# AechPro/Prism

Hardware: NVIDIA B200
Metric: PER sampled transitions/s (4 new steps ingested -> sample -> 3-step gather -> DQN update -> priority write-back, per learner iteration) (higher is better)
Workload: dtype f32

## Files before the change

### include/prism_b200.h

```cpp
#ifndef PRISM_B200_H
#define PRISM_B200_H

#include <stdint.h>

#ifdef __cplusplus
extern "C" {
#endif

#define PB_ABI_VERSION 2

enum {
    PB_OK = 0,
    PB_E_ARG = -1,
    PB_E_CAPACITY = -2,
    PB_E_UNSUPPORTED = -3,
    PB_E_POOL = -4
};

enum {
    PB_ST_EMPTY = 1,
    PB_ST_PSUM_NONPOS = 2,
    PB_ST_PMIN_NONPOS = 4
};

// ... 157 lines not shown
int pb_ens_q_loss_total(int B, int A, int K, const float *q_cur, const float *q_next_online, const float *q_next_target,
                        const long long *action, const float *ret, const float *gdn, const uint8_t *nonterminal,
                        float loss_weight, const float *row_weight, float grad_scale, float *loss_out, float *grad_q_cur,
                        const float *dist, float q_scale, const float *q_offset, float *total_out, float *td_out,
                        unsigned int *ticket, void *stream);

int pb_ids_select(int N, int A, int K, int Nq, const float *q, const float *z, float lambda,
                  float eps, float rho_lower_bound, long long *action_out, float *scores_out,
                  void *stream);

int pb_greedy_select(int N, int A, int K, const float *q, long long *action_out, void *stream);

#define PB_ADAM_MAX_PARTIALS 4096
int pb_pack_grads_parity(int n_tensors, const long long *table, float scale, float *flat,
                         const unsigned long long *epoch, long long stride, float *partial_scratch,
                         long long *step_count, int *n_partials_out_h, void *stream);
int pb_pack_grads(int n_tensors, const long long *table, float scale, float *flat,
                  float *partial_scratch, long long *step_count, int *n_partials_out_h,
                  void *stream);
int pb_grad_sumsq(long long n, const float *grad, float *partial_scratch, long long *step_count,
                  int *n_partials_out_h, void *stream);
int pb_adam_clip_apply(long long n, float *param, const float *grad, float *exp_avg,
                       float *exp_avg_sq, const long long *step_count, float lr, float beta1,
                       float beta2, float adam_eps, float max_grad_norm,
                       const float *partial_scratch, int n_partials, float *norm_out,
                       void *stream);
long long pb_adam_fused_max_n(void);
int pb_adam_fused_step(int n_tensors, const long long *table, float scale, long long n, float *param, float *grad,
                       float *exp_avg, float *exp_avg_sq, long long *step_count, float lr, float beta1, float beta2,
                       float adam_eps, float max_grad_norm, float *partial_scratch, float *norm_out, void *stream);
int pb_adam_clip_step(long long n, float *param, const float *grad, float *exp_avg, float *exp_avg_sq,
                      long long *step_count, float lr, float beta1, float beta2, float adam_eps,
                      float max_grad_norm, float *norm_out, float *partial_scratch, void *stream);

#define PB_OPT_ADAM 0
#define PB_OPT_RMSPROP 1
#define PB_OPT_RMSPROP_CENTERED 2
#define PB_OPT_SGD 3
long long pb_opt_fused_max_n(int rule);
int pb_opt_fused_step(int rule, int n_tensors, const long long *table, float scale, long long n, float *param, float *grad,
                      float *m, float *v, long long *step_count, float lr, float h1, float h2, float eps,
                      float max_grad_norm, float *partial_scratch, float *norm_out, void *stream);
int pb_opt_clip_apply(int rule, long long n, float *param, const float *grad, float *m, float *v,
                      const long long *step_count, float lr, float h1, float h2, float eps, float max_grad_norm,
                      const float *partial_scratch, int n_partials, float *norm_out, void *stream);

int pb_conv3x3_relu_supported(int H, int W, int C, int OC);
int pb_conv3x3_relu_fwd(int B, int H, int W, int C, int OC, const float *x, const float *w,
                        const float *bias, float *out, void *stream);
int pb_conv3x3_relu_bwd_groups(int B);
int pb_conv3x3_relu_bwd(int B, int H, int W, int C, int OC, const float *x, const float *out,
                        const float *dout, float *partial_scratch, float *dw, float *db,
                        void *stream);

int pb_linear_fwd(int K, int M, int N, int J, const float *X, long long x_head_stride, const float *W,
                  const float *b, int act, float *Y, void *stream);
int pb_linear_bwd_input(int K, int M, int N, int J, const float *dY, const float *Ymask, const float *W,
                        int sum_heads, float *dX, void *stream);
int pb_linear_bwd_weight(int K, int M, int N, int J, const float *dY, const float *Ymask, const float *X,
                         long long x_head_stride, float *dW, float *db, void *stream);
int pb_gemm_trace(int enable, unsigned long long *out, int n_out);

int pb_tc_gemm_supported(int M, int N, int K, long long lda, long long ldb, long long ldc);
int pb_tc_gemm(int batch, int kbatches, int M, int N, int K,
               const float *A, int a_major, long long lda, long long a_bs,
               const float *B, int b_major, long long ldb, long long b_bs,
               const float *bias, long long bias_bs, int act,
               const float *mul, int mul_rows, long long ld_mul,
               float *C, long long ldc, long long c_bs,
               float *workspace, long long workspace_floats, int split_mode, void *stream);
int pb_linear_fwd_tc_supported(int M, int N, int J);
int pb_linear_fwd_tc(int K, int M, int N, int J, const float *X, long long x_head_stride, const float *W,
                     const float *b, int act, float *Y, void *stream);

int pb_iqn_phi_bwd(int n, int B, int F, const float *dh, const float *phi, const float *x, float *dpre, float *dx,
                   float *dbias_partial, void *stream);

#define PB_PEER_MAX 8
typedef struct pb_peer_group {
    int world, rank;
    float *grad[PB_PEER_MAX];
    float *reduced[PB_PEER_MAX];
    unsigned long long *flags[PB_PEER_MAX];
    double *norm_parts[PB_PEER_MAX];
    unsigned char *state[PB_PEER_MAX];
    unsigned long long *epoch;
    unsigned int *status;
    unsigned long long timeout_ns;
    long long grad_stride;
} pb_peer_group;
int pb_peer_alloc(long long bytes, void **ptr);
int pb_peer_free(void *ptr);
int pb_optimizer_preload(void);
int pb_peer_preload(void);
int pb_peer_export(const void *ptr, void *handle64);
int pb_peer_open(const void *handle64, void **ptr);
int pb_peer_close(void *ptr);
int pb_peer_barrier(const pb_peer_group *g, void *stream);
int pb_peer_state_allgather(const pb_peer_group *g, const void *state64, void *all_state_out, void *stream);
long long pb_peer_slice(long long n, int world);
int pb_peer_reduce_scatter(const pb_peer_group *g, long long n, float *partial_scratch, long long *step_count, void *stream);
int pb_peer_pull_sum(const pb_peer_group *g, long long n, float *partial_scratch, long long *step_count,
                     int *n_partials_out_h, void *stream);
int pb_peer_adam(const pb_peer_group *g, long long n, float *param, float *exp_avg, float *exp_avg_sq,
                 const long long *step_count, float lr, float beta1, float beta2, float adam_eps, float max_grad_norm,
                 float *norm_out, float *grad_out, void *stream);
// ... 78 lines not shown
```

### prism_b200/_lib.py

```python
import ctypes as C
import os

from . import build as _build

_LIB = None


class PbError(RuntimeError):
    pass


class pb_per_state(C.Structure):
    _fields_ = [
        ("len", C.c_longlong), ("seq", C.c_longlong), ("max_priority", C.c_float), ("p_sum", C.c_float),
        ("p_min", C.c_float), ("status", C.c_int), ("batch_max", C.c_float), ("owned_lo", C.c_int),
        ("owned_n", C.c_int), ("pad", C.c_int * 5),
    ]


class pb_tree(C.Structure):
    _fields_ = [
        ("sum", C.c_void_p), ("min", C.c_void_p), ("owner", C.c_void_p), ("counters", C.c_void_p),
        ("state", C.c_void_p),
        ("capacity", C.c_longlong), ("size", C.c_longlong), ("alpha", C.c_float), ("eps_f32", C.c_float),
# ... 41 lines not shown
    "pb_error_string": [_I],
    "pb_launch_count": [],
    "pb_event_create": [C.POINTER(C.c_void_p)],
    "pb_event_destroy": [_P],
    "pb_event_record": [_P, _P],
    "pb_event_synchronize": [_P],
    "pb_stream_wait_event": [_P, _P],
    "pb_copy_h2d_async": [_P, _P, _LL, _P],
    "pb_staged_copy_submit": [_P, _P, _P, _P, _LL, _P, _P],
    "pb_copy_d2h_async": [_P, _P, _LL, _P],
    "pb_copy_d2d_async": [_P, _P, _LL, _P],
    "pb_tree_layout": [_LL, C.POINTER(C.c_longlong), C.POINTER(C.c_longlong), C.POINTER(C.c_longlong),
                       C.POINTER(C.c_longlong), C.POINTER(C.c_int)],
    "pb_tree_init": [_TREE, _P],
    "pb_tree_export": [_TREE, _P, _P, _P],
    "pb_tree_trace": [_I, _P, _I],
    "pb_gemm_trace": [_I, _P, _I],
    "pb_tree_sample_batches": [_TREE, _LL, _LL, _P, _I, _F, _P, _P, _P, _P],
    "pb_tree_build": [_TREE, _P, _LL, _P],
    "pb_tree_stats": [_TREE, _P],
    "pb_tree_set_leaves": [_TREE, _LL, _P, _P, _I, _P],
    "pb_tree_update_priority": [_TREE, _LL, _P, _P, _I, _P],
    "pb_tree_extend": [_TREE, _LL, _P, _P],
    "pb_tree_scan": [_TREE, _LL, _P, _P, _P],
    "pb_tree_sample": [_TREE, _LL, _P, _I, _F, _P, _P, _P, _P],
    "pb_tree_sample_global": [_TREE, _I, _I, _P, _LL, _P, _F, _P, _P, _P, _P],
    "pb_store_extend_plan": [_LL, _LL, _I, _LL, _LL, _P, _P, _P, _P, _P, _P],
    "pb_store_scatter": [_STORE, _LL, _P, _P, _P, _P],
    "pb_select_copy_f64": [_P, _P, _P, _P, _LL, _LL, _P],
    "pb_store_scatter_dbuf": [_STORE, _LL, _P, _P, _P, _P, _P, _P, _P, _P],
    "pb_store_gather": [_STORE, _LL, _P, _P, _P, _P, _P, _P, _P, _P],
    "pb_store_nstep": [_STORE, _LL, _P, _P, _P, _P, _P, _P, _P],
    "pb_iqn_cos_basis": [_LL, _I, _P, _P, _P],
    "pb_iqn_qh_loss": [_I, _I, _I, _I, _P, _P, _P, _P, _P, _P, _P, _P, _F, _F, _P, _F, _P, _P, _P],
    "pb_ens_q_loss": [_I, _I, _I, _P, _P, _P, _P, _P, _P, _P, _F, _P, _F, _P, _P, _P],
    "pb_ens_q_loss_total": [_I, _I, _I, _P, _P, _P, _P, _P, _P, _P, _F, _P, _F, _P, _P, _P, _F, _P, _P, _P, _P, _P],
    "pb_ids_select": [_I, _I, _I, _I, _P, _P, _F, _F, _F, _P, _P, _P],
    "pb_greedy_select": [_I, _I, _I, _P, _P, _P],
    "pb_adam_clip_step": [_LL, _P, _P, _P, _P, _P, _F, _F, _F, _F, _F, _P, _P, _P],
    "pb_adam_fused_max_n": [],
    "pb_adam_fused_step": [_I, _P, _F, _LL, _P, _P, _P, _P, _P, _F, _F, _F, _F, _F, _P, _P, _P],
    "pb_pack_grads": [_I, _P, _F, _P, _P, _P, _P, _P],
    "pb_pack_grads_parity": [_I, _P, _F, _P, _P, _LL, _P, _P, _P, _P],
    "pb_grad_sumsq": [_LL, _P, _P, _P, _P, _P],
    "pb_adam_clip_apply": [_LL, _P, _P, _P, _P, _P, _F, _F, _F, _F, _F, _P, _I, _P, _P],
    "pb_opt_fused_max_n": [_I],
    "pb_opt_fused_step": [_I, _I, _P, _F, _LL, _P, _P, _P, _P, _P, _F, _F, _F, _F, _F, _P, _P, _P],
    "pb_opt_clip_apply": [_I, _LL, _P, _P, _P, _P, _P, _F, _F, _F, _F, _F, _P, _I, _P, _P],
    "pb_loss_combine": [_I, _P, _P, _P, _F, _P, _P, _P, _P],
    "pb_conv3x3_relu_supported": [_I, _I, _I, _I],
    "pb_conv3x3_relu_fwd": [_I, _I, _I, _I, _I, _P, _P, _P, _P, _P],
    "pb_conv3x3_relu_bwd_groups": [_I],
    "pb_conv3x3_relu_bwd": [_I, _I, _I, _I, _I, _P, _P, _P, _P, _P, _P, _P],
    "pb_linear_fwd": [_I, _I, _I, _I, _P, _LL, _P, _P, _I, _P, _P],
    "pb_peer_alloc": [_LL, C.POINTER(C.c_void_p)],
    "pb_peer_free": [_P],
    "pb_peer_preload": [],
    "pb_optimizer_preload": [],
    "pb_peer_export": [_P, _P],
    "pb_peer_open": [_P, C.POINTER(C.c_void_p)],
    "pb_peer_close": [_P],
    "pb_peer_barrier": [_PEER, _P],
    "pb_peer_state_allgather": [_PEER, _P, _P, _P],
    "pb_peer_slice": [_LL, _I],
    "pb_peer_reduce_scatter": [_PEER, _LL, _P, _P, _P],
    "pb_peer_pull_sum": [_PEER, _LL, _P, _P, C.POINTER(C.c_int), _P],
    "pb_peer_adam": [_PEER, _LL, _P, _P, _P, _P, _F, _F, _F, _F, _F, _P, _P, _P],
    "pb_peer_allreduce_adam_max_n": [],
    "pb_peer_allreduce_adam": [_PEER, _LL, _P, _P, _P, _P, _F, _F, _F, _F, _F, _P, _P, _P],
    "pb_peer_allreduce_opt_max_n": [_I],
    "pb_peer_allreduce_opt": [_I, _PEER, _LL, _P, _P, _P, _P, _F, _F, _F, _F, _F, _P, _P, _P],
    "pb_peer_opt": [_I, _PEER, _LL, _P, _P, _P, _P, _F, _F, _F, _F, _F, _P, _P, _P],
    "pb_peer_state_put": [_PEER, _P, _P],
    "pb_peer_trace": [_I, _P, _I],
    "pb_tree_sample_global_peer": [_TREE, _PEER, _LL, _P, _F, _P, _P, _P, _P],
    "pb_uniform_init": [_P, _LL, _LL, _I, _P],
    "pb_uniform_extend": [_P, _LL, _LL, _P],
    "pb_uniform_sample": [_P, _LL, _P, _I, _P, _P, _P],
    "pb_uniform_sample_global": [_P, _I, _I, _P, _LL, _P, _P, _P, _P, _P],
    "pb_uniform_sample_global_peer": [_P, _PEER, _LL, _P, _P, _P, _P, _P],
    "pb_layer_norm_supported": [_LL, _I],
    "pb_layer_norm_bwd_blocks": [_LL, _I],
    "pb_layer_norm_fwd": [_LL, _I, _F, _P, _P, _P, _P, _P, _P, _P],
    "pb_layer_norm_bwd": [_LL, _I, _P, _P, _P, _P, _P, _P, _P, _P, _P, _P],
    "pb_layer_norm_grouped_fwd": [_I, _LL, _LL, _I, _F, _P, _P, _P, _P, _P, _P, _P],
    "pb_layer_norm_grouped_bwd_blocks": [_I, _LL, _I],
    "pb_layer_norm_grouped_bwd": [_I, _LL, _LL, _I, _P, _P, _P, _P, _P, _P, _P, _P, _P, _P],
    "pb_narrow_linear_supported": [_LL, _I, _I],
    "pb_narrow_linear_bwd_blocks": [_LL],
    "pb_narrow_linear_fwd": [_I, _LL, _I, _I, _P, _LL, _P, _P, _P, _P],
    "pb_narrow_linear_bwd": [_I, _LL, _I, _I, _P, _LL, _P, _P, _P, _P, _P, _P, _P],
    "pb_narrow_linear_bwd_reduce": [_I, _LL, _I, _I, _P, _P, _P, _P],
    "pb_sum_heads": [_I, _LL, _P, _P, _P],
    "pb_iqn_draw_cos_basis": [_LL, _I, _P, _P, _P, _P],
    "pb_relu_bwd_bias_strips": [_LL],
    "pb_relu_bwd_bias": [_I, _LL, _I, _P, _P, _P, _P, _P, _P],
    "pb_theil_chunks": [_LL],
    "pb_theil_fwd": [_I, _I, _I, _P, _P, _P, _P, _P],
    "pb_theil_bwd": [_I, _I, _I, _P, _P, _P, _P, _P],
    "pb_iqn_phi_bwd": [_I, _I, _I, _P, _P, _P, _P, _P, _P, _P],
    "pb_tc_gemm_supported": [_I, _I, _I, _LL, _LL, _LL],
    "pb_tc_gemm": [_I, _I, _I, _I, _I, _P, _I, _LL, _LL, _P, _I, _LL, _LL, _P, _LL, _I, _P, _I, _LL, _P, _LL, _LL, _P, _LL, _I, _P],
    "pb_linear_fwd_tc_supported": [_I, _I, _I],
    "pb_linear_fwd_tc": [_I, _I, _I, _I, _P, _LL, _P, _P, _I, _P, _P],
    "pb_linear_bwd_input": [_I, _I, _I, _I, _P, _P, _P, _I, _P, _P],
    "pb_linear_bwd_weight": [_I, _I, _I, _I, _P, _P, _P, _LL, _P, _P, _P],
# ... 62 lines not shown
```

### prism_b200/agents/ops.py

```python
import collections

import torch

from .. import _lib

ROUTES = collections.Counter()


def route_counts(reset=False):
    out = dict(ROUTES)
    if reset:
        ROUTES.clear()
    return out


def fallthrough_count():
    return sum(v for k, v in ROUTES.items() if k.startswith("fallthrough"))


def _c(t, dtype=torch.float32):
    if t.dtype != dtype:
        t = t.to(dtype)
    return t if t.is_contiguous() else t.contiguous()

# ... 639 lines not shown
        _lib.require_cuda(ref, "tables")
        lib, stream, dev = _lib.load(), _stream(ref), ref.device
        B = action.numel()
        action_c, ret_c, gamma_c = _c(action, torch.int64).view(-1), _c(ret).view(-1), _c(gamma).view(-1)
        nt = None if nonterm is None else nonterm.contiguous().view(-1).view(torch.uint8)
        w_c = None if w is None else _c(w).view(-1)
        dist = mse = gz = gq = None
        if z_cur is not None:
            zc = _c(z_cur)
            dist = torch.empty(B, dtype=torch.float32, device=dev)
            gz = torch.empty_like(zc)
            _lib.check(lib.pb_iqn_qh_loss(B, T, Tp, zc.shape[-1], zc.data_ptr(), _c(tau).view(-1).data_ptr(),
                                          _c(z_on).data_ptr(), _c(z_tg).data_ptr(), action_c.data_ptr(),
                                          ret_c.data_ptr(), gamma_c.data_ptr(), _lib.ptr(nt), float(kappa),
                                          float(dist_weight), _lib.ptr(w_c), 1.0 / B, dist.data_ptr(), gz.data_ptr(),
                                          stream), "pb_iqn_qh_loss")
        total = torch.empty((), dtype=torch.float32, device=dev)
        td = torch.empty(B, dtype=torch.float32, device=dev)
        if q_cur is not None:
            qc = _c(q_cur)
            K, _, A = qc.shape
            mse = torch.empty(B, dtype=torch.float32, device=dev)
            gq = torch.empty_like(qc)
            _lib.check(lib.pb_ens_q_loss_total(B, A, K, qc.data_ptr(), _c(q_on).data_ptr(), _c(q_tg).data_ptr(),
                                               action_c.data_ptr(), ret_c.data_ptr(), gamma_c.data_ptr(), _lib.ptr(nt), 1.0,
                                               _lib.ptr(w_c), float(q_weight) / B, mse.data_ptr(), gq.data_ptr(),
                                               _lib.ptr(dist), float(q_weight), _lib.ptr(q_offset), total.data_ptr(),
                                               td.data_ptr(), _loss_ticket(dev).data_ptr(), stream), "pb_ens_q_loss_total")
        else:
            _lib.check(lib.pb_loss_combine(B, _lib.ptr(dist), None, _lib.ptr(w_c), float(q_weight),
                                           _lib.ptr(q_offset), total.data_ptr(), td.data_ptr(), stream), "pb_loss_combine")
        ctx.save_for_backward(gz, gq)
        ctx.set_materialize_grads(False)
        outs = (total, dist if dist is not None else td.new_empty(0), mse if mse is not None else td.new_empty(0), td)
        ctx.mark_non_differentiable(*outs[1:])
        return outs

    @staticmethod
    def backward(ctx, g_total, *_):
        gz, gq = ctx.saved_tensors
        if g_total is None:
            return (None,) * 18
        if UNIT_TOTAL_GRAD:
            return (gz, gq) + (None,) * 16
        return (None if gz is None else gz * g_total, None if gq is None else gq * g_total) + (None,) * 16


def fused_total_loss(z_cur, q_cur, tau, z_on, z_tg, q_on, q_tg, action, ret, gamma, nonterm, w, q_offset, T, Tp,
                     kappa, dist_weight, q_weight):
    return _FusedTotalLoss.apply(z_cur, q_cur, tau, z_on, z_tg, q_on, q_tg, action, ret, gamma, nonterm, w, q_offset,
                                 T, Tp, kappa, dist_weight, q_weight)


class _ConvEmbed(torch.autograd.Function):

    @staticmethod
    def forward(ctx, x, weight, bias):
        _lib.require_cuda(x, "x")
        B, H, W, C = x.shape
        OC = weight.shape[0]
        xc, wc, bc = _c(x), _c(weight), (None if bias is None else _c(bias))
        out = torch.empty(B, OC * (H - 2) * (W - 2), dtype=torch.float32, device=x.device)
        _lib.check(_lib.load().pb_conv3x3_relu_fwd(B, H, W, C, OC, xc.data_ptr(), wc.data_ptr(), _lib.ptr(bc),
                                                   out.data_ptr(), _stream(x)), "pb_conv3x3_relu_fwd")
        ctx.dims = (B, H, W, C, OC)
        ctx.has_bias = bias is not None
        ctx.save_for_backward(xc, out)
        return out

    @staticmethod
    def backward(ctx, dout):
        xc, out = ctx.saved_tensors
        B, H, W, C, OC = ctx.dims
        lib = _lib.load()
        dout = _c(dout)
        groups = lib.pb_conv3x3_relu_bwd_groups(B)
        scratch = torch.empty(groups * (OC * C * 9 + OC), dtype=torch.float32, device=dout.device)
        dw = torch.empty(OC, C, 3, 3, dtype=torch.float32, device=dout.device)
        db = torch.empty(OC, dtype=torch.float32, device=dout.device) if ctx.has_bias else None
        _lib.check(lib.pb_conv3x3_relu_bwd(B, H, W, C, OC, xc.data_ptr(), out.data_ptr(), dout.data_ptr(),
                                           scratch.data_ptr(), dw.data_ptr(), _lib.ptr(db), _stream(dout)),
                   "pb_conv3x3_relu_bwd")
        if TRACE_MARK is not None:
            TRACE_MARK("bwd:conv3x3")
        return None, dw, db


def conv3x3_relu_flatten(x, weight, bias):
    return _ConvEmbed.apply(x, weight, bias)
```

### prism_b200/csrc/conv.cu

```cuda
#include "common.cuh"
#include <stdlib.h>

namespace {

using namespace pb;

constexpr int MAX_X = 16 * 16 * 16;
constexpr int MAX_W = 32 * 16 * 9;
constexpr int MAX_OUT = 32 * 14 * 14;

struct ConvDims { int B, H, W, C, OC, OH, OW; };

constexpr int OCG = 8;

__host__ __device__ inline int frame_pitch(int W) { return ((W + 7) / 16) * 16 + 8; }

__device__ __forceinline__ unsigned div_magic(int d) { return 0xFFFFFFFFu / (unsigned)d + 1u; }
__device__ __forceinline__ int frame_slot(int i, int H, int W, int C, int P, unsigned mC, unsigned mW)
{
    const int pix = C == 1 ? i : (int)__umulhi((unsigned)i, mC), c = i - pix * C;
    const int y = (int)__umulhi((unsigned)pix, mW), x = pix - y * W;
    return (c * H + y) * P + x;
}

__global__ void __launch_bounds__(256) conv3x3_relu_fwd_kernel(ConvDims d, const float *__restrict__ x,
                                                               const float *__restrict__ w,
                                                               const float *__restrict__ bias, float *__restrict__ out)
{
    pdl_wait();
    pdl_trigger();
    extern __shared__ __align__(16) float sm[];
    const int nx = d.H * d.W * d.C, ocp = (d.OC + OCG - 1) / OCG * OCG, taps = d.C * 9;
    const int P = frame_pitch(d.W), cstride = d.H * P;
    const unsigned mC = div_magic(d.C), mW = div_magic(d.W), mO = div_magic(ocp);
    float *sw = sm, *sx = sm + taps * ocp;
    const int b = blockIdx.x;
    const float *xb = x + (size_t)b * nx;
    {
        const int nwp = taps * ocp;
        for (int i0 = threadIdx.x; i0 < nx || i0 < nwp; i0 += 8 * blockDim.x) {
            float fx[8], fw[8];
#pragma unroll
            for (int u = 0; u < 8; ++u) {
                const int i = i0 + u * blockDim.x;
                fx[u] = i < nx ? xb[i] : 0.0f;
                const int tap = (int)__umulhi((unsigned)i, mO), oc = i - tap * ocp;
                fw[u] = (i < nwp && oc < d.OC) ? w[oc * taps + tap] : 0.0f;
            }
#pragma unroll
            for (int u = 0; u < 8; ++u) {
                const int i = i0 + u * blockDim.x;
                if (i < nx) sx[frame_slot(i, d.H, d.W, d.C, P, mC, mW)] = fx[u];
                if (i < nwp) sw[i] = fw[u];
            }
// ... 55 lines not shown
#pragma unroll
        for (int q = 0; q < 8; ++q) {
            const int u = threadIdx.x + q * blockDim.x;
            if (u >= ne) break;
            float a0 = 0.0f, a1 = 0.0f, a2 = 0.0f, a3 = 0.0f;
            if (u < nw) {
                const int tap = u / d.OC, oc = u - tap * d.OC, c = tap / 9, k = tap - c * 9, ky = k / 3, kx = k - ky * 3;
                const float *g = sg + oc;
                for (int y = 0; y < d.OH; ++y) {
                    const float *gy = g + y * d.OW * d.OC, *xy = sx + ((y + ky) * d.W + kx) * d.C + c;
                    int xx = 0;
                    for (; xx + 3 < d.OW; xx += 4) {
                        a0 = fmaf(gy[xx * d.OC], xy[xx * d.C], a0);
                        a1 = fmaf(gy[(xx + 1) * d.OC], xy[(xx + 1) * d.C], a1);
                        a2 = fmaf(gy[(xx + 2) * d.OC], xy[(xx + 2) * d.C], a2);
                        a3 = fmaf(gy[(xx + 3) * d.OC], xy[(xx + 3) * d.C], a3);
                    }
                    for (; xx < d.OW; ++xx) a0 = fmaf(gy[xx * d.OC], xy[xx * d.C], a0);
                }
            } else {
                const float *g = sg + (u - nw);
                int p = 0;
                for (; p + 3 < plane; p += 4) {
                    a0 += g[p * d.OC]; a1 += g[(p + 1) * d.OC]; a2 += g[(p + 2) * d.OC]; a3 += g[(p + 3) * d.OC];
                }
                for (; p < plane; ++p) a0 += g[p * d.OC];
            }
            acc[q] += (a0 + a1) + (a2 + a3);
        }
    }
#pragma unroll
    for (int q = 0; q < 8; ++q) {
        const int u = threadIdx.x + q * blockDim.x;
        if (u >= ne) break;
        int e = u;
        if (u < nw) { const int tap = u / d.OC, oc = u - tap * d.OC; e = oc * taps + tap; }
        partial[(size_t)blockIdx.x * ne + e] = acc[q];
    }
}

__device__ __forceinline__ void conv_mma_tf32(float (&d)[4], const uint32_t (&a)[4], const uint32_t (&b)[2])
{
    asm volatile("mma.sync.aligned.m16n8k8.row.col.f32.tf32.tf32.f32 {%0,%1,%2,%3}, {%4,%5,%6,%7}, {%8,%9}, {%0,%1,%2,%3};"
                 : "+f"(d[0]), "+f"(d[1]), "+f"(d[2]), "+f"(d[3])
                 : "r"(a[0]), "r"(a[1]), "r"(a[2]), "r"(a[3]), "r"(b[0]), "r"(b[1]));
}
__device__ __forceinline__ void conv_split_tf32(float x, uint32_t &hi, uint32_t &lo)
{
    hi = __float_as_uint(x) & 0xFFFFE000u;
    lo = __float_as_uint(x - __uint_as_float(hi));
}

constexpr int CM_WARPS = 4;
constexpr int CM_MAX_NT = 12;
constexpr int CM_GSTRIDE = 68;

template <int NT>
__global__ void __launch_bounds__(CM_WARPS * 32) conv3x3_relu_bwd_mma_kernel(ConvDims d, const float *__restrict__ x,
                                                                            const float *__restrict__ out,
                                                                            const float *__restrict__ dout,
                                                                            float *__restrict__ partial, int n_groups)
{
    pdl_wait();
    pdl_trigger();
    extern __shared__ float sm[];
    constexpr int NTW = (NT + CM_WARPS - 1) / CM_WARPS;
    const int nx = d.H * d.W * d.C, plane = d.OH * d.OW, taps = d.C * 9, ne = 16 * taps + 16;
    const int P = frame_pitch(d.W), cstride = d.H * P;
    const unsigned mC = div_magic(d.C), mW = div_magic(d.W);
    const int warp = threadIdx.x >> 5, lane = threadIdx.x & 31, gq = lane >> 2, tq = lane & 3;
    float *sx = sm, *sg = sx + cstride * d.C;
    int *pos_off = reinterpret_cast<int *>(sg + 16 * CM_GSTRIDE), *tap_off = pos_off + plane;
    for (int p = threadIdx.x; p < plane; p += blockDim.x) pos_off[p] = (p / d.OW) * P + (p % d.OW);
    for (int tp = threadIdx.x; tp < NT * 8; tp += blockDim.x) {
        int v = -2;
        if (tp < taps) { const int c = tp / 9, k = tp - c * 9; v = c * cstride + (k / 3) * P + (k % 3); }
        else if (tp == taps) v = -1;
        tap_off[tp] = v;
    }
    float cf[NTW][4];
#pragma unroll
    for (int j = 0; j < NTW; ++j) cf[j][0] = cf[j][1] = cf[j][2] = cf[j][3] = 0.0f;
    const int g = blockIdx.x;
    for (int b = g; b < d.B; b += n_groups) {
        __syncthreads();
        const float *xb = x + (size_t)b * nx, *ob = out + (size_t)b * 16 * plane, *gb = dout + (size_t)b * 16 * plane;
        for (int i0 = threadIdx.x; i0 < nx; i0 += 8 * blockDim.x) {
            float v[8];
#pragma unroll
            for (int u = 0; u < 8; ++u) { const int i = i0 + u * blockDim.x; v[u] = i < nx ? xb[i] : 0.0f; }
#pragma unroll
            for (int u = 0; u < 8; ++u) {
                const int i = i0 + u * blockDim.x;
                if (i < nx) sx[frame_slot(i, d.H, d.W, d.C, P, mC, mW)] = v[u];
            }
        }
        for (int i0 = threadIdx.x; i0 < 16 * plane; i0 += 8 * blockDim.x) {
            float vo[8], vg[8];
#pragma unroll
            for (int u = 0; u < 8; ++u) {
                const int i = i0 + u * blockDim.x;
                vo[u] = i < 16 * plane ? ob[i] : 0.0f;
                vg[u] = i < 16 * plane ? gb[i] : 0.0f;
            }
#pragma unroll
            for (int u = 0; u < 8; ++u) {
                const int i = i0 + u * blockDim.x;
                if (i < 16 * plane) {
                    const int oc = i / plane, p = i - oc * plane;
                    sg[oc * CM_GSTRIDE + p] = vo[u] > 0.0f ? vg[u] : 0.0f;
                }
            }
        }
        __syncthreads();
        int toff[NTW];
#pragma unroll
        for (int j = 0; j < NTW; ++j) { const int nt = warp + j * CM_WARPS; toff[j] = nt < NT ? tap_off[nt * 8 + gq] : -2; }
        for (int k0 = 0; k0 < plane; k0 += 8) {
            uint32_t ah[4], al[4];
            conv_split_tf32(sg[gq * CM_GSTRIDE + k0 + tq], ah[0], al[0]);
            conv_split_tf32(sg[(gq + 8) * CM_GSTRIDE + k0 + tq], ah[1], al[1]);
            conv_split_tf32(sg[gq * CM_GSTRIDE + k0 + tq + 4], ah[2], al[2]);
            conv_split_tf32(sg[(gq + 8) * CM_GSTRIDE + k0 + tq + 4], ah[3], al[3]);
            const int p0 = pos_off[k0 + tq], p1 = pos_off[k0 + tq + 4];
#pragma unroll
            for (int j = 0; j < NTW; ++j) {
                if (warp + j * CM_WARPS >= NT) break;
                const int to = toff[j];
                const float b0 = to >= 0 ? sx[p0 + to] : (to == -1 ? 1.0f : 0.0f);
                const float b1 = to >= 0 ? sx[p1 + to] : (to == -1 ? 1.0f : 0.0f);
                uint32_t bh[2], bl[2];
                conv_split_tf32(b0, bh[0], bl[0]);
                conv_split_tf32(b1, bh[1], bl[1]);
                conv_mma_tf32(cf[j], al, bh);
                conv_mma_tf32(cf[j], ah, bl);
                conv_mma_tf32(cf[j], ah, bh);
            }
        }
    }
    if (g < n_groups) {
        float *pg = partial + (size_t)g * ne;
#pragma unroll
        for (int j = 0; j < NTW; ++j) {
            const int nt = warp + j * CM_WARPS;
            if (nt >= NT) break;
#pragma unroll
            for (int q = 0; q < 4; ++q) {
                const int oc = gq + (q >> 1) * 8, tp = nt * 8 + 2 * tq + (q & 1);
                if (tp < taps) pg[oc * taps + tp] = cf[j][q];
                else if (tp == taps) pg[16 * taps + oc] = cf[j][q];
            }
        }
    }
}

__global__ void __launch_bounds__(256) conv_bwd_reduce_kernel(int n_groups, int nw, int n_bias,
                                                              const float *__restrict__ partial,
                                                              float *__restrict__ dw, float *__restrict__ db)
{
    pdl_wait();
    pdl_trigger();
    const int e = (blockIdx.x * blockDim.x + threadIdx.x) >> 5, ne = nw + n_bias;
    if (e >= ne) return;
    float a = 0.0f;
    for (int g = lane_id(); g < n_groups; g += 32) a += partial[(size_t)g * ne + e];
    a = warp_sum(a);
    if (lane_id() == 0) {
        if (e < nw) dw[e] = a; else if (db) db[e - nw] = a;
    }
}

size_t fwd_smem(const ConvDims &d)
{
    const int ocp = (d.OC + OCG - 1) / OCG * OCG;
    return sizeof(float) * (size_t)(d.H * frame_pitch(d.W) * d.C + ocp * d.C * 9);
}
size_t fma_bwd_smem(const ConvDims &d) { return sizeof(float) * (size_t)(d.H * d.W * d.C + d.OC * d.OH * d.OW); }

int check_dims(const ConvDims &d)
{
    if (d.B <= 0 || d.H < 3 || d.W < 3 || d.C <= 0 || d.OC <= 0) return PB_E_ARG;
    const long long H = d.H, W = d.W, C = d.C, OC = d.OC;
    if (H * W * C > MAX_X || OC * C * 9 > MAX_W || OC * (H - 2) * (W - 2) > MAX_OUT) return PB_E_UNSUPPORTED;
    if (OC * C * 9 + OC > 8 * 256) return PB_E_UNSUPPORTED;
    if (fwd_smem(d) > 48 * 1024 || fma_bwd_smem(d) > 48 * 1024) return PB_E_UNSUPPORTED;
    return PB_OK;
}

}

extern "C" {

int pb_conv3x3_relu_supported(int H, int W, int C, int OC)
{
    const ConvDims d = {1, H, W, C, OC, H - 2, W - 2};
    return check_dims(d) == PB_OK ? 1 : 0;
}

int pb_conv3x3_relu_fwd(int B, int H, int W, int C, int OC, const float *x, const float *w, const float *bias,
                        float *out, void *stream)
{
    ConvDims d = {B, H, W, C, OC, H - 2, W - 2};
    int rc = check_dims(d);
    if (rc) return rc;
    if (!x || !w || !out) return PB_E_ARG;
    const int ocp = (OC + 7) / 8 * 8;
    const size_t smem = fwd_smem(d);
    const int items = d.OH * d.OW * (ocp / 8);
    const int threads = items >= 256 ? 256 : (items + 31) / 32 * 32;
    PB_LAUNCH_PDL_CHAIN(conv3x3_relu_fwd_kernel, (unsigned)B, threads, smem, stream, d, x, w, bias, out);
    return PB_OK;
}

int pb_conv3x3_relu_bwd_groups(int B) { return B < 296 ? B : 296; }

int pb_conv3x3_relu_bwd(int B, int H, int W, int C, int OC, const float *x, const float *out, const float *dout,
                        float *partial_scratch, float *dw, float *db, void *stream)
{
    ConvDims d = {B, H, W, C, OC, H - 2, W - 2};
    int rc = check_dims(d);
    if (rc) return rc;
    if (!x || !out || !dout || !partial_scratch || !dw) return PB_E_ARG;
    const int groups = pb_conv3x3_relu_bwd_groups(B);
    const int ne = OC * C * 9 + OC;
    {
        static int mma_ok = -1;
        if (mma_ok < 0) { const char *e = getenv("PB_CONV_MMA"); mma_ok = (e && e[0] == '0') ? 0 : 1; }
        const int plane = d.OH * d.OW, nt = (C * 9 + 1 + 7) / 8;
        const size_t msmem = sizeof(float) * (size_t)(H * frame_pitch(W) * C + 16 * CM_GSTRIDE + plane + nt * 8);
        if (mma_ok && OC == 16 && (plane % 8) == 0 && plane <= 64 && nt >= 5 && nt <= CM_MAX_NT && msmem <= 48 * 1024) {
            const unsigned grid = (unsigned)groups;
#define PB_CONV_MMA_CASE(NTV)                                                                                      \
            case NTV: PB_LAUNCH_PDL_CHAIN(conv3x3_relu_bwd_mma_kernel<NTV>, grid, CM_WARPS * 32, msmem, stream, d, x, out, \
                                          dout, partial_scratch, groups); break;
            switch (nt) {
                PB_CONV_MMA_CASE(5) PB_CONV_MMA_CASE(6) PB_CONV_MMA_CASE(7) PB_CONV_MMA_CASE(8) PB_CONV_MMA_CASE(9)
                PB_CONV_MMA_CASE(10) PB_CONV_MMA_CASE(11) PB_CONV_MMA_CASE(12)
                default: goto fma_path;
            }
#undef PB_CONV_MMA_CASE
            PB_LAUNCH_PDL_CHAIN(conv_bwd_reduce_kernel, (unsigned)((ne + 7) / 8), 256, 0, stream, groups, OC * C * 9, OC,
                                partial_scratch, dw, db);
            return PB_OK;
        }
    }
fma_path:
    const size_t smem = fma_bwd_smem(d);
    const int ne_all = OC * C * 9 + OC;
    const int bthreads = ne_all > 256 ? 512 : 256;
    PB_LAUNCH_PDL_CHAIN(conv3x3_relu_bwd_kernel, (unsigned)groups, bthreads, smem, stream, d, x, out, dout, partial_scratch);
    PB_LAUNCH_PDL_CHAIN(conv_bwd_reduce_kernel, (unsigned)((ne + 7) / 8), 256, 0, stream, groups, OC * C * 9, OC,
              partial_scratch, dw, db);
    return PB_OK;
}

}
```

### profiles/kernel_chain.py

```python
import os
import sys

import torch

sys.path.insert(0, os.path.dirname(os.path.dirname(os.path.abspath(__file__))))
from prism_b200.agents import ops

DEV = "cuda:0"
N = 40


def timed(name, fn, reps=30):
    s = torch.cuda.Stream()
    with torch.cuda.stream(s):
        for _ in range(3):
            fn()
    torch.cuda.synchronize()
    g = torch.cuda.CUDAGraph()
    with torch.cuda.graph(g):
        for _ in range(N):
            fn()
    for _ in range(5):
        g.replay()
    e0, e1 = torch.cuda.Event(enable_timing=True), torch.cuda.Event(enable_timing=True)
# ... 2 lines not shown
    for _ in range(reps):
        g.replay()
    e1.record()
    torch.cuda.synchronize()
    print("%-58s %7.2f us per call" % (name, e0.elapsed_time(e1) * 1e3 / (reps * N)))


def main():
    torch.manual_seed(0)
    B, C = 256, 6
    obs = torch.rand(B, 10, 10, C, device=DEV)
    cw, cb = torch.randn(16, C, 3, 3, device=DEV) * 0.1, torch.zeros(16, device=DEV)
    w1, b1 = torch.randn(1, 256, 1024, device=DEV) * 0.03, torch.zeros(1, 256, device=DEV)
    w2, b2 = torch.randn(1, 6, 256, device=DEV) * 0.05, torch.zeros(1, 6, device=DEV)
    with torch.no_grad():
        emb = ops.conv3x3_relu_flatten(obs, cw, cb)
        h = ops.linear_heads(emb, w1, b1, relu=True)
        timed("conv3x3+relu+flatten fwd (256 x 10x10x6 -> 1024)", lambda: ops.conv3x3_relu_flatten(obs, cw, cb))
        timed("linear 1024 -> 256 + relu fwd (ours)", lambda: ops.linear_heads(emb, w1, b1, relu=True))
        timed("linear 1024 -> 256 + relu fwd (library addmm + relu)",
              lambda: torch.relu(torch.addmm(b1[0], emb, w1[0].t())))
        timed("narrow 256 -> 6 fwd", lambda: ops.linear_heads(h[0] if h.dim() == 3 else h, w2, b2))
    import ctypes as C
    from prism_b200 import _lib
    lib = _lib.load()
    names = ["first chunk staged", "K loop done", "partial tile written", "cluster barrier", "split-K sum + epilogue",
             "exit barrier"]
    for label, fn in (("forward 256 x 256 x 1024", lambda: ops.linear_heads(emb, w1, b1, relu=True)),):
        with torch.no_grad():
            for _ in range(3):
                fn()
            lib.pb_gemm_trace(1, None, 0)
            fn()
        out = (C.c_ulonglong * 8)()
        lib.pb_gemm_trace(0, out, 8)
        print("phases of one launch, %s (latest CTA, us after the earliest CTA start):" % label)
        for k, nm in enumerate(names):
            print("   %6.2f  %s" % ((out[k + 1] - out[0]) / 1e3, nm))
    embg = emb.clone().requires_grad_(False)
    w1g, b1g = w1.clone().requires_grad_(True), b1.clone().requires_grad_(True)
    embr = emb.clone().requires_grad_(True)
    gy = torch.randn(1, 256, 256, device=DEV)

    def lin_fb():
        y = ops.linear_heads(embr, w1g, b1g, relu=True)
        torch.autograd.grad(y, (embr, w1g, b1g), gy)
    timed("linear fwd + dgrad + wgrad (two branches)", lin_fb)
    cwg, cbg = cw.clone().requires_grad_(True), cb.clone().requires_grad_(True)
    ge = torch.randn(B, 1024, device=DEV)

    def conv_fb():
        y = ops.conv3x3_relu_flatten(obs, cwg, cbg)
        torch.autograd.grad(y, (cwg, cbg), ge)
    timed("conv fwd + bwd (mma) + reduce", conv_fb)


if __name__ == "__main__":
    main()
```

Measured before the change: 3.424 million.

## Fuse conv backward reduction into MMA kernel via cluster DSMEM and ticket

The tensor-core conv weight-gradient kernel now runs in thread-block clusters of 8. It reduces per-CTA partials across the cluster through distributed shared memory, and the last cluster to arrive, found through an atomic ticket counter, sums the cluster rows and writes dW/db directly. This removes the separate reduce kernel launch, and the next sample's inputs are prefetched into registers while MMAs run. The scratch buffer is also cached, zero-initialised, so the ticket counters persist. The cost is added cluster synchronisation, a serial final reduction done by one cluster, and reliance on the tickets resetting themselves correctly.

```diff
diff --git a/include/prism_b200.h b/include/prism_b200.h
--- a/include/prism_b200.h
+++ b/include/prism_b200.h
@@ -233,6 +233,7 @@
 int pb_conv3x3_relu_bwd(int B, int H, int W, int C, int OC, const float *x, const float *out,
                         const float *dout, float *partial_scratch, float *dw, float *db,
                         void *stream);
+int pb_conv_trace(int enable, unsigned long long *out, int n_out);
 
 int pb_linear_fwd(int K, int M, int N, int J, const float *X, long long x_head_stride, const float *W,
                   const float *b, int act, float *Y, void *stream);
diff --git a/prism_b200/_lib.py b/prism_b200/_lib.py
--- a/prism_b200/_lib.py
+++ b/prism_b200/_lib.py
@@ -117,6 +117,7 @@
     "pb_conv3x3_relu_fwd": [_I, _I, _I, _I, _I, _P, _P, _P, _P, _P],
     "pb_conv3x3_relu_bwd_groups": [_I],
     "pb_conv3x3_relu_bwd": [_I, _I, _I, _I, _I, _P, _P, _P, _P, _P, _P, _P],
+    "pb_conv_trace": [_I, _P, _I],
     "pb_linear_fwd": [_I, _I, _I, _I, _P, _LL, _P, _P, _I, _P, _P],
     "pb_peer_alloc": [_LL, C.POINTER(C.c_void_p)],
     "pb_peer_free": [_P],
diff --git a/prism_b200/agents/ops.py b/prism_b200/agents/ops.py
--- a/prism_b200/agents/ops.py
+++ b/prism_b200/agents/ops.py
@@ -715,6 +715,19 @@
                                  T, Tp, kappa, dist_weight, q_weight)
 
 
+_CONV_SCRATCH = {}
+
+
+def _conv_scratch(device, n):
+    key = (device, n)
+    t = _CONV_SCRATCH.get(key)
+    if t is None:
+        t = torch.zeros(n, dtype=torch.float32, device=device)
+        if not torch.cuda.is_current_stream_capturing():
+            _CONV_SCRATCH[key] = t
+    return t
+
+
 class _ConvEmbed(torch.autograd.Function):
 
     @staticmethod
@@ -738,7 +751,7 @@
         lib = _lib.load()
         dout = _c(dout)
         groups = lib.pb_conv3x3_relu_bwd_groups(B)
-        scratch = torch.empty(groups * (OC * C * 9 + OC), dtype=torch.float32, device=dout.device)
+        scratch = _conv_scratch(dout.device, groups * (OC * C * 9 + OC))
         dw = torch.empty(OC, C, 3, 3, dtype=torch.float32, device=dout.device)
         db = torch.empty(OC, dtype=torch.float32, device=dout.device) if ctx.has_bias else None
         _lib.check(lib.pb_conv3x3_relu_bwd(B, H, W, C, OC, xc.data_ptr(), out.data_ptr(), dout.data_ptr(),
diff --git a/prism_b200/csrc/conv.cu b/prism_b200/csrc/conv.cu
--- a/prism_b200/csrc/conv.cu
+++ b/prism_b200/csrc/conv.cu
@@ -1,5 +1,8 @@
 #include "common.cuh"
+#include <cooperative_groups.h>
 #include <stdlib.h>
+
+namespace cg = cooperative_groups;
 
 namespace {
 
@@ -161,70 +164,93 @@
 }
 
 constexpr int CM_WARPS = 4;
+constexpr int CM_THREADS = CM_WARPS * 32;
+constexpr int CM_CLUSTER = 8;
+constexpr int CM_MAX_CTAS = 256;
+constexpr int CM_MAX_ROWS = CM_MAX_CTAS / CM_CLUSTER;
 constexpr int CM_MAX_NT = 12;
 constexpr int CM_GSTRIDE = 68;
+constexpr int CM_XPT = (3 * 66 * 10 + CM_THREADS - 1) / CM_THREADS;
+constexpr int CM_GPT = 16 * 64 / CM_THREADS;
+
+__device__ unsigned long long g_conv_trace[8];
+__device__ int g_conv_trace_on;
+__device__ __forceinline__ void conv_mark(int on, int slot)
+{
+    if (on && threadIdx.x == 0) {
+        const unsigned long long v = global_ns();
+        if (slot == 0) asm volatile("red.relaxed.gpu.global.min.u64 [%0], %1;" :: "l"(g_conv_trace), "l"(v) : "memory");
+        else asm volatile("red.relaxed.gpu.global.max.u64 [%0], %1;" :: "l"(g_conv_trace + slot), "l"(v) : "memory");
+    }
+}
 
 template <int NT>
-__global__ void __launch_bounds__(CM_WARPS * 32) conv3x3_relu_bwd_mma_kernel(ConvDims d, const float *__restrict__ x,
-                                                                            const float *__restrict__ out,
-                                                                            const float *__restrict__ dout,
-                                                                            float *__restrict__ partial, int n_groups)
+__global__ void __launch_bounds__(CM_THREADS) conv3x3_relu_bwd_mma_kernel(ConvDims d, const float *__restrict__ x,
+                                                                         const float *__restrict__ out,
+                                                                         const float *__restrict__ dout,
+                                                                         float *__restrict__ partial,
+                                                                         unsigned *__restrict__ ticket,
+                                                                         float *__restrict__ dw, float *__restrict__ db)
 {
     pdl_wait();
     pdl_trigger();
-    extern __shared__ float sm[];
+    extern __shared__ __align__(16) float sm[];
+    __shared__ int s_last;
     constexpr int NTW = (NT + CM_WARPS - 1) / CM_WARPS;
-    const int nx = d.H * d.W * d.C, plane = d.OH * d.OW, taps = d.C * 9, ne = 16 * taps + 16;
+    const int tr_on = __ldg(&g_conv_trace_on);
+    conv_mark(tr_on, 0);
+    const int nx = d.H * d.W * d.C, plane = d.OH * d.OW, ng = 16 * plane, taps = d.C * 9, nw = 16 * taps, ne = nw + 16;
     const int P = frame_pitch(d.W), cstride = d.H * P;
-    const unsigned mC = div_magic(d.C), mW = div_magic(d.W);
-    const int warp = threadIdx.x >> 5, lane = threadIdx.x & 31, gq = lane >> 2, tq = lane & 3;
+    const unsigned mC = div_magic(d.C), mW = div_magic(d.W), mP = div_magic(plane);
+    const int tid = threadIdx.x, warp = tid >> 5, lane = tid & 31, gq = lane >> 2, tq = lane & 3;
     float *sx = sm, *sg = sx + cstride * d.C;
     int *pos_off = reinterpret_cast<int *>(sg + 16 * CM_GSTRIDE), *tap_off = pos_off + plane;
-    for (int p = threadIdx.x; p < plane; p += blockDim.x) pos_off[p] = (p / d.OW) * P + (p % d.OW);
-    for (int tp = threadIdx.x; tp < NT * 8; tp += blockDim.x) {
+    for (int p = tid; p < plane; p += CM_THREADS) pos_off[p] = (p / d.OW) * P + (p % d.OW);
+    for (int tp = tid; tp < NT * 8; tp += CM_THREADS) {
         int v = -2;
         if (tp < taps) { const int c = tp / 9, k = tp - c * 9; v = c * cstride + (k / 3) * P + (k % 3); }
         else if (tp == taps) v = -1;
         tap_off[tp] = v;
     }
+    float fx[CM_XPT], fo[CM_GPT], fg[CM_GPT];
+    auto fetch = [&](int b) {
+        const float *xb = x + (size_t)b * nx, *ob = out + (size_t)b * ng, *gb = dout + (size_t)b * ng;
+#pragma unroll
+        for (int u = 0; u < CM_XPT; ++u) { const int i = tid + u * CM_THREADS; fx[u] = i < nx ? xb[i] : 0.0f; }
+#pragma unroll
+        for (int u = 0; u < CM_GPT; ++u) {
+            const int i = tid + u * CM_THREADS;
+            fo[u] = i < ng ? ob[i] : 0.0f;
+            fg[u] = i < ng ? gb[i] : 0.0f;
+        }
+    };
+    const int G = gridDim.x;
+    if (blockIdx.x < d.B) fetch(blockIdx.x);
+    __syncthreads();
+    int toff[NTW];
+#pragma unroll
+    for (int j = 0; j < NTW; ++j) { const int nt = warp + j * CM_WARPS; toff[j] = nt < NT ? tap_off[nt * 8 + gq] : -2; }
     float cf[NTW][4];
 #pragma unroll
     for (int j = 0; j < NTW; ++j) cf[j][0] = cf[j][1] = cf[j][2] = cf[j][3] = 0.0f;
-    const int g = blockIdx.x;
-    for (int b = g; b < d.B; b += n_groups) {
+    for (int b = blockIdx.x; b < d.B; b += G) {
         __syncthreads();
-        const float *xb = x + (size_t)b * nx, *ob = out + (size_t)b * 16 * plane, *gb = dout + (size_t)b * 16 * plane;
-        for (int i0 = threadIdx.x; i0 < nx; i0 += 8 * blockDim.x) {
-            float v[8];
-#pragma unroll
-            for (int u = 0; u < 8; ++u) { const int i = i0 + u * blockDim.x; v[u] = i < nx ? xb[i] : 0.0f; }
-#pragma unroll
-            for (int u = 0; u < 8; ++u) {
-                const int i = i0 + u * blockDim.x;
-                if (i < nx) sx[frame_slot(i, d.H, d.W, d.C, P, mC, mW)] = v[u];
-            }
-        }
-        for (int i0 = threadIdx.x; i0 < 16 * plane; i0 += 8 * blockDim.x) {
-            float vo[8], vg[8];
-#pragma unroll
-            for (int u = 0; u < 8; ++u) {
-                const int i = i0 + u * blockDim.x;
-                vo[u] = i < 16 * plane ? ob[i] : 0.0f;
-                vg[u] = i < 16 * plane ? gb[i] : 0.0f;
-            }
-#pragma unroll
-            for (int u = 0; u < 8; ++u) {
-                const int i = i0 + u * blockDim.x;
-                if (i < 16 * plane) {
-                    const int oc = i / plane, p = i - oc * plane;
-                    sg[oc * CM_GSTRIDE + p] = vo[u] > 0.0f ? vg[u] : 0.0f;
-                }
+#pragma unroll
+        for (int u = 0; u < CM_XPT; ++u) {
+            const int i = tid + u * CM_THREADS;
+            if (i < nx) sx[frame_slot(i, d.H, d.W, d.C, P, mC, mW)] = fx[u];
+        }
+#pragma unroll
+        for (int u = 0; u < CM_GPT; ++u) {
+            const int i = tid + u * CM_THREADS;
+            if (i < ng) {
+                const int oc = (int)__umulhi((unsigned)i, mP), p = i - oc * plane;
+                sg[oc * CM_GSTRIDE + p] = fo[u] > 0.0f ? fg[u] : 0.0f;
             }
         }
         __syncthreads();
-        int toff[NTW];
-#pragma unroll
-        for (int j = 0; j < NTW; ++j) { const int nt = warp + j * CM_WARPS; toff[j] = nt < NT ? tap_off[nt * 8 + gq] : -2; }
+        if (b == (int)blockIdx.x) conv_mark(tr_on, 1);
+        if (b + G < d.B) fetch(b + G);
         for (int k0 = 0; k0 < plane; k0 += 8) {
             uint32_t ah[4], al[4];
             conv_split_tf32(sg[gq * CM_GSTRIDE + k0 + tq], ah[0], al[0]);
@@ -247,20 +273,77 @@
             }
         }
     }
-    if (g < n_groups) {
-        float *pg = partial + (size_t)g * ne;
-#pragma unroll
-        for (int j = 0; j < NTW; ++j) {
-            const int nt = warp + j * CM_WARPS;
-            if (nt >= NT) break;
-#pragma unroll
-            for (int q = 0; q < 4; ++q) {
-                const int oc = gq + (q >> 1) * 8, tp = nt * 8 + 2 * tq + (q & 1);
-                if (tp < taps) pg[oc * taps + tp] = cf[j][q];
-                else if (tp == taps) pg[16 * taps + oc] = cf[j][q];
-            }
-        }
-    }
+    conv_mark(tr_on, 2);
+    float *red = sm;
+    __syncthreads();
+#pragma unroll
+    for (int j = 0; j < NTW; ++j) {
+        const int nt = warp + j * CM_WARPS;
+        if (nt >= NT) break;
+#pragma unroll
+        for (int q = 0; q < 4; ++q) {
+            const int oc = gq + (q >> 1) * 8, tp = nt * 8 + 2 * tq + (q & 1);
+            if (tp < taps) red[oc * taps + tp] = cf[j][q];
+            else if (tp == taps) red[nw + oc] = cf[j][q];
+        }
+    }
+    cg::cluster_group cluster = cg::this_cluster();
+    cluster.sync();
+    const int rank = (int)cluster.block_rank(), cl = blockIdx.x / CM_CLUSTER, n_cl = G / CM_CLUSTER;
+    const int per = (ne + CM_CLUSTER - 1) / CM_CLUSTER, e0 = rank * per, e1 = min(ne, e0 + per);
+    for (int e = e0 + tid; e < e1; e += CM_THREADS) {
+        float v[CM_CLUSTER];
+#pragma unroll
+        for (int r = 0; r < CM_CLUSTER; ++r) v[r] = cluster.map_shared_rank(red, r)[e];
+        float s = v[0];
+#pragma unroll
+        for (int r = 1; r < CM_CLUSTER; ++r) s += v[r];
+        partial[(size_t)cl * ne + e] = s;
+    }
+    asm volatile("barrier.cluster.arrive.release.aligned;" ::: "memory");
+    conv_mark(tr_on, 3);
+    __syncthreads();
+    if (tid == 0) {
+        unsigned t;
+        asm volatile("atom.acq_rel.gpu.global.add.u32 %0, [%1], 1;" : "=r"(t) : "l"(ticket + rank) : "memory");
+        s_last = t == (unsigned)(n_cl - 1);
+        if (s_last) ticket[rank] = 0u;
+    }
+    __syncthreads();
+    if (s_last) {
+        for (int e = e0 + tid; e < e1; e += CM_THREADS) {
+            float v[CM_MAX_ROWS];
+#pragma unroll
+            for (int c = 0; c < CM_MAX_ROWS; ++c) v[c] = c < n_cl ? __ldcg(partial + (size_t)c * ne + e) : 0.0f;
+            float s = v[0];
+#pragma unroll
+            for (int c = 1; c < CM_MAX_ROWS; ++c) s += v[c];
+            if (e < nw) dw[e] = s; else if (db) db[e - nw] = s;
+        }
+        conv_mark(tr_on, 4);
+    }
+    asm volatile("barrier.cluster.wait.acquire.aligned;" ::: "memory");
+}
+
+template <int NT>
+int launch_conv_bwd_mma(const ConvDims &d, unsigned grid, size_t smem, void *stream, const float *x, const float *out,
+                        const float *dout, float *partial, unsigned *ticket, float *dw, float *db)
+{
+    cudaLaunchConfig_t cfg = {};
+    cfg.gridDim = dim3(grid);
+    cfg.blockDim = dim3(CM_THREADS);
+    cfg.dynamicSmemBytes = smem;
+    cfg.stream = (cudaStream_t)stream;
+    cudaLaunchAttribute attr[2];
+    attr[0].id = cudaLaunchAttributeClusterDimension;
+    attr[0].val.clusterDim.x = CM_CLUSTER; attr[0].val.clusterDim.y = 1; attr[0].val.clusterDim.z = 1;
+    attr[1].id = cudaLaunchAttributeProgrammaticStreamSerialization;
+    attr[1].val.programmaticStreamSerializationAllowed = 1;
+    cfg.attrs = attr;
+    cfg.numAttrs = pb_pdl_chain_enabled() ? 2 : 1;
+    cudaError_t e = cudaLaunchKernelEx(&cfg, conv3x3_relu_bwd_mma_kernel<NT>, d, x, out, dout, partial, ticket, dw, db);
+    g_pb_launches.fetch_add(1, std::memory_order_relaxed);
+    return e == cudaSuccess ? PB_OK : (int)e;
 }
 
 __global__ void __launch_bounds__(256) conv_bwd_reduce_kernel(int n_groups, int nw, int n_bias,
@@ -321,7 +404,8 @@
     return PB_OK;
 }
 
-int pb_conv3x3_relu_bwd_groups(int B) { return B < 296 ? B : 296; }
+static int fma_groups(int B) { return B < 296 ? B : 296; }
+int pb_conv3x3_relu_bwd_groups(int B) { return fma_groups(B) + 1; }
 
 int pb_conv3x3_relu_bwd(int B, int H, int W, int C, int OC, const float *x, const float *out, const float *dout,
                         float *partial_scratch, float *dw, float *db, void *stream)
@@ -330,7 +414,7 @@
     int rc = check_dims(d);
     if (rc) return rc;
     if (!x || !out || !dout || !partial_scratch || !dw) return PB_E_ARG;
-    const int groups = pb_conv3x3_relu_bwd_groups(B);
+    const int groups = fma_groups(B);
     const int ne = OC * C * 9 + OC;
     {
         static int mma_ok = -1;
@@ -338,29 +422,42 @@
         const int plane = d.OH * d.OW, nt = (C * 9 + 1 + 7) / 8;
         const size_t msmem = sizeof(float) * (size_t)(H * frame_pitch(W) * C + 16 * CM_GSTRIDE + plane + nt * 8);
         if (mma_ok && OC == 16 && (plane % 8) == 0 && plane <= 64 && nt >= 5 && nt <= CM_MAX_NT && msmem <= 48 * 1024) {
-            const unsigned grid = (unsigned)groups;
+            const int ctas = (B + CM_CLUSTER - 1) / CM_CLUSTER * CM_CLUSTER;
+            const unsigned grid = (unsigned)(ctas < CM_MAX_CTAS ? ctas : CM_MAX_CTAS);
+            unsigned *ticket = reinterpret_cast<unsigned *>(partial_scratch + (size_t)groups * ne);
 #define PB_CONV_MMA_CASE(NTV)                                                                                      \
-            case NTV: PB_LAUNCH_PDL_CHAIN(conv3x3_relu_bwd_mma_kernel<NTV>, grid, CM_WARPS * 32, msmem, stream, d, x, out, \
-                                          dout, partial_scratch, groups); break;
+            case NTV: return launch_conv_bwd_mma<NTV>(d, grid, msmem, stream, x, out, dout, partial_scratch, ticket, dw, db);
             switch (nt) {
                 PB_CONV_MMA_CASE(5) PB_CONV_MMA_CASE(6) PB_CONV_MMA_CASE(7) PB_CONV_MMA_CASE(8) PB_CONV_MMA_CASE(9)
                 PB_CONV_MMA_CASE(10) PB_CONV_MMA_CASE(11) PB_CONV_MMA_CASE(12)
-                default: goto fma_path;
+                default: break;
             }
 #undef PB_CONV_MMA_CASE
-            PB_LAUNCH_PDL_CHAIN(conv_bwd_reduce_kernel, (unsigned)((ne + 7) / 8), 256, 0, stream, groups, OC * C * 9, OC,
-                                partial_scratch, dw, db);
-            return PB_OK;
-        }
-    }
-fma_path:
+        }
+    }
     const size_t smem = fma_bwd_smem(d);
-    const int ne_all = OC * C * 9 + OC;
-    const int bthreads = ne_all > 256 ? 512 : 256;
+    const int bthreads = ne > 256 ? 512 : 256;
     PB_LAUNCH_PDL_CHAIN(conv3x3_relu_bwd_kernel, (unsigned)groups, bthreads, smem, stream, d, x, out, dout, partial_scratch);
     PB_LAUNCH_PDL_CHAIN(conv_bwd_reduce_kernel, (unsigned)((ne + 7) / 8), 256, 0, stream, groups, OC * C * 9, OC,
               partial_scratch, dw, db);
     return PB_OK;
 }
 
-}
+int pb_conv_trace(int enable, unsigned long long *out, int n_out)
+{
+    unsigned long long host[8];
+    cudaError_t e = cudaDeviceSynchronize();
+    if (e != cudaSuccess) return (int)e;
+    e = cudaMemcpyFromSymbol(host, g_conv_trace, sizeof(host));
+    if (e != cudaSuccess) return (int)e;
+    if (out) for (int k = 0; k < n_out && k < 8; ++k) out[k] = host[k];
+    for (int k = 0; k < 8; ++k) host[k] = 0;
+    host[0] = ~0ULL;
+    e = cudaMemcpyToSymbol(g_conv_trace, host, sizeof(host));
+    if (e != cudaSuccess) return (int)e;
+    const int on = enable ? 1 : 0;
+    e = cudaMemcpyToSymbol(g_conv_trace_on, &on, sizeof(on));
+    return e == cudaSuccess ? PB_OK : (int)e;
+}
+
+}
diff --git a/profiles/kernel_chain.py b/profiles/kernel_chain.py
--- a/profiles/kernel_chain.py
+++ b/profiles/kernel_chain.py
@@ -78,7 +78,26 @@
     def conv_fb():
         y = ops.conv3x3_relu_flatten(obs, cwg, cbg)
         torch.autograd.grad(y, (cwg, cbg), ge)
-    timed("conv fwd + bwd (mma) + reduce", conv_fb)
+    timed("conv fwd + bwd (mma, one launch)", conv_fb)
+    nc = obs.shape[-1]
+    y = ops.conv3x3_relu_flatten(obs, cw, cb)
+    scratch = torch.zeros(lib.pb_conv3x3_relu_bwd_groups(B) * (16 * nc * 9 + 16), device=DEV)
+    dwc, dbc = torch.empty(16, nc, 3, 3, device=DEV), torch.empty(16, device=DEV)
+
+    def conv_b():
+        _lib.check(lib.pb_conv3x3_relu_bwd(B, 10, 10, nc, 16, obs.data_ptr(), y.data_ptr(), ge.data_ptr(),
+                                           scratch.data_ptr(), dwc.data_ptr(), dbc.data_ptr(),
+                                           C.c_void_p(torch.cuda.current_stream().cuda_stream)), "pb_conv3x3_relu_bwd")
+    timed("conv bwd alone (256 x 10x10x6, 16 filters)", conv_b)
+    for _ in range(3):
+        conv_b()
+    lib.pb_conv_trace(1, None, 0)
+    conv_b()
+    out = (C.c_ulonglong * 8)()
+    lib.pb_conv_trace(0, out, 8)
+    print("phases of one launch, conv backward 256 x 10x10x6 (latest CTA, us after the earliest CTA start):")
+    for k, nm in enumerate(["first sample staged", "MMAs done", "partial written", "dW / db written"]):
+        print("   %6.2f  %s" % ((out[k + 1] - out[0]) / 1e3, nm))
 
 
 if __name__ == "__main__":
```

New measurement: 3.422 million (median of 6 runs). Within noise of the previous version (-0.0%).
